# EBI-Metagenomics/deciphon-old

Measured on AMD Instinct MI355X. Metric: Gcell-updates/sec, higher is better.
Workload: dtype f32

## Files before the change

deciphon-old_amd/csrc/dcp_qlane.hip:

```cpp
#include "dcp_kernels.h"

#include <hip/hip_runtime.h>
#include <type_traits>

namespace
{
constexpr int NC = DCP_NCODES;

#ifndef DCP_QLANE_RECOMPUTE_B
#define DCP_QLANE_RECOMPUTE_B 1
#endif
constexpr bool kRecomputeB = DCP_QLANE_RECOMPUTE_B != 0;
#ifndef DCP_QLANE_WD
#define DCP_QLANE_WD 5
#endif
constexpr unsigned kWD = DCP_QLANE_WD;
constexpr unsigned kPlanes = kRecomputeB ? 3u : 4u;
#ifndef DCP_QLANE_DIAG
#define DCP_QLANE_DIAG 0
#endif

#ifndef DCP_QL_WPLANE
#define DCP_QL_WPLANE 1
#endif
#ifndef DCP_QL_IN16
#define DCP_QL_IN16 1
#endif
#ifndef DCP_QL_EM
#define DCP_QL_EM 1
#endif
constexpr bool kWPlane = DCP_QL_WPLANE != 0, kIn16 = DCP_QL_IN16 != 0, kEM = DCP_QL_EM != 0;

typedef float const __attribute__((address_space(4))) cfloat;
__device__ __forceinline__ cfloat *as_const(float const *p)
{
    return (cfloat *)(unsigned long long)p;
}

__device__ __forceinline__ float ninf() { return -__builtin_inff(); }
__device__ __forceinline__ float mx3(float a, float b, float c) { return fmaxf(fmaxf(a, b), c); }
__device__ __forceinline__ float mx5(float a, float b, float c, float d, float e)
{
    return mx3(mx3(a, b, c), d, e);
}

template <int G> struct QState
{
    float P[5][4 * G];
    float Q[5][4 * G];
    float PN[5], PR[5];
    float PJ[5], PC[5];
};

struct LaneXt
{
    float RR, SB, SN, NN, NB, ET, EC, CC, CT, EB, EJ, JJ, JB;
};

struct SweepOut
{
    float E, C, Rn;
};

template <int G> struct TileTrans
{
    float ent[4 * G], mi[4 * G], ii[4 * G];
    float mm[4 * G + 1], im[4 * G + 1], dm[4 * G + 1], md[4 * G + 1], dd[4 * G + 1];
};

template <int G> __device__ __forceinline__ void load_tile_trans(TileTrans<G> &t, cfloat *tt)
{
    constexpr int KT = 4 * G;
#pragma unroll
    for (int k = 0; k < KT; ++k)
    {
        t.ent[k] = tt[k * 8 + DCP_T_ENTRY];
        t.mi[k] = tt[k * 8 + DCP_T_MI];
        t.ii[k] = tt[k * 8 + DCP_T_II];
    }
#pragma unroll
    for (int k = 1; k <= KT; ++k)
    {
        t.mm[k] = tt[k * 8 + DCP_T_MM];
        t.im[k] = tt[k * 8 + DCP_T_IM];
        t.dm[k] = tt[k * 8 + DCP_T_DM];
        t.md[k] = tt[k * 8 + DCP_T_MD];
        t.dd[k] = tt[k * 8 + DCP_T_DD];
    }
    t.mm[0] = t.im[0] = t.dm[0] = t.md[0] = t.dd[0] = 0.0f;
}

struct RowIn
{
    float4 e0[5];
    float eI[5], eN[5];
};

template <int G, bool ROWS>
__device__ __forceinline__ void stage_tile_image(float *tabM, dcp_qlane_args const &a, dcp_ql_prof const &pm, unsigned t,
                                                 unsigned first, unsigned stride)
{
    constexpr unsigned N4 = (unsigned)(G * NC);
    float4 *dst = reinterpret_cast<float4 *>(tabM);
    if constexpr (!ROWS)
    {
        float4 const *__restrict__ src = reinterpret_cast<float4 const *>(a.emis_tiles + pm.tile_off + (size_t)t * (N4 * 4u));
        for (unsigned i = first; i < N4; i += stride)
            dst[i] = src[i];
    }
    else
    {
        float const *__restrict__ rows = a.emis_tiles + pm.tile_off + t * (4u * (unsigned)G);
        unsigned const ldk = pm.ldk, M = pm.core_size;
        for (unsigned i = first; i < N4; i += stride)
        {
            unsigned const grp = i / (unsigned)NC, code = i - grp * (unsigned)NC;
            float4 v = make_float4(ninf(), ninf(), ninf(), ninf());
            if (t * (4u * (unsigned)G) + grp * 4u < M)
                v = *reinterpret_cast<float4 const *>(rows + (size_t)code * ldk + grp * 4u);
            dst[i] = v;
        }
    }
}

__device__ __forceinline__ float ld_off(float const *base, unsigned boff)
{
    return *reinterpret_cast<float const *>(reinterpret_cast<char const *>(base) + boff);
}
typedef uint32_t const __attribute__((address_space(1))) *gu32_ptr;
typedef uint16_t const __attribute__((address_space(1))) *gu16_ptr;
typedef char const __attribute__((address_space(1))) *gchar_ptr;
__device__ __forceinline__ void st_off(float *base, unsigned boff, float v)
{
    *reinterpret_cast<float *>(reinterpret_cast<char *>(base) + boff) = v;
}

struct Ring
{
    float B[5], Xm[5], Xd[5], Em[5];
};

enum
{
    IO_HBM = 1,
    IO_LDS = 2
};
constexpr unsigned kRD = 16;
constexpr unsigned kRLanes = 256;
constexpr unsigned kRingPlaneBytes = kRD * kRLanes * 4u;
#ifndef DCP_Q2_SKEW
#define DCP_Q2_SKEW 4
#endif
#ifndef DCP_Q2_HYST
#define DCP_Q2_HYST 1
#endif
#ifndef DCP_Q2_SLEEP
#define DCP_Q2_SLEEP 2
#endif
#ifndef DCP_Q2_PRIO
#define DCP_Q2_PRIO 0
#endif
#ifndef DCP_Q2_STAGEMAP
#define DCP_Q2_STAGEMAP 1
#endif
constexpr unsigned kRingSkew = DCP_Q2_SKEW;
constexpr unsigned kRingHyst = DCP_Q2_HYST;
typedef float __attribute__((address_space(3))) lds_float;
typedef unsigned __attribute__((address_space(3))) lds_uint;

typedef char __attribute__((address_space(3))) lds_char;

struct LdsLink
{
    lds_char *base;
    unsigned my_flag;
    unsigned peer_flag;
    unsigned seen;
};
constexpr unsigned kL2TabIN = 43648u;
constexpr unsigned kL2FlagP = kL2TabIN + 2u * 1364u * 4u;
constexpr unsigned kL2FlagC = kL2FlagP + kRLanes * 4u;
constexpr unsigned kL2Null = kL2FlagC + kRLanes * 4u;
constexpr unsigned kL2Task = kL2Null + kRLanes * 4u;
constexpr unsigned kL2Abort = kL2Task + 4u;
constexpr unsigned kL2Err = kL2Task + 8u;
constexpr unsigned kL2Tab1 = 65536u;
constexpr unsigned kL2Ring = 7u * kRingPlaneBytes;
constexpr unsigned kL2Bytes = kL2Ring + 3u * kRingPlaneBytes;
static_assert(kL2Task + 16u <= kL2Tab1 && kL2Tab1 + kL2TabIN <= kL2Ring && kL2Bytes == 160u * 1024u, "LDS layout");
static_assert((kL2Ring & (kRingPlaneBytes - 1u)) == 0u, "ring slots are addressed by OR");
static_assert(kRD >= 12u, "a shorter ring can deadlock the two stages (five-row hand-shake groups)");

__device__ __forceinline__ void compiler_fence() { asm volatile("" ::: "memory"); }
#define DCP_ISA_MARK(name) asm volatile("; " name ::: "memory")
__device__ __forceinline__ unsigned flag_load(lds_uint *flag)
{
    return __hip_atomic_load(flag, __ATOMIC_RELAXED, __HIP_MEMORY_SCOPE_WORKGROUP);
}
__device__ __forceinline__ void flag_store(lds_uint *flag, unsigned v)
{
    __hip_atomic_store(flag, v, __ATOMIC_RELAXED, __HIP_MEMORY_SCOPE_WORKGROUP);
}
#ifndef DCP_Q2_BOUND
#define DCP_Q2_BOUND 1
#endif
constexpr unsigned kRingSpinBound = 1u << 23;
constexpr unsigned kRingPoison = 0x7fffff00u;
__device__ __forceinline__ unsigned ring_wait(LdsLink const &lk, unsigned need)
{
    lds_uint *flag = (lds_uint *)(lk.base + lk.peer_flag);
    unsigned v = __builtin_amdgcn_readfirstlane(flag_load(flag));
#if DCP_Q2_BOUND
    unsigned spins = 0;
#pragma nounroll
    while (v < need)
    {
        __builtin_amdgcn_s_sleep(DCP_Q2_SLEEP);
        v = __builtin_amdgcn_readfirstlane(flag_load(flag));
        if (__builtin_expect(++spins == kRingSpinBound, 0))
        {
            typedef unsigned __attribute__((address_space(1))) *gerr_ptr;
            gerr_ptr const err = *(gerr_ptr __attribute__((address_space(3))) *)(lk.base + kL2Err);
            __hip_atomic_store(err, 1u, __ATOMIC_RELAXED, __HIP_MEMORY_SCOPE_AGENT);
            flag_store((lds_uint *)(lk.base + kL2Abort), 1u);
            flag_store(flag, kRingPoison);
            v = kRingPoison;
            __builtin_amdgcn_s_waitcnt(0x0070);
        }
    }
#else
    while (v < need)
    {
        __builtin_amdgcn_s_sleep(DCP_Q2_SLEEP);
        v = __builtin_amdgcn_readfirstlane(flag_load(flag));
    }
#endif
    DCP_ISA_MARK("DCP_RING_ACQUIRED");
    return v;
}
__device__ __forceinline__ float ring_ld(LdsLink const &lk, unsigned rowoff, unsigned plane)
{
    return *(lds_float *)(lk.base + ((rowoff & (kRingPlaneBytes - 1u)) | kL2Ring) + plane * kRingPlaneBytes);
}
__device__ __forceinline__ void ring_st(LdsLink const &lk, unsigned rowoff, unsigned plane, float v)
{
    *(lds_float *)(lk.base + ((rowoff & (kRingPlaneBytes - 1u)) | kL2Ring) + plane * kRingPlaneBytes) = v;
}
__device__ __forceinline__ void ring_publish(LdsLink const &lk, unsigned rowoff, unsigned row)
{
    flag_store((lds_uint *)(lk.base + lk.my_flag + (rowoff & (kRLanes * 4u - 1u))), row);
}

template <bool FIRST>
__device__ __forceinline__ void ring_fetch_x(Ring &r, int slot, float const *pXm, float const *pXd,
                                             float const *pEm, unsigned off)
{
    if constexpr (!FIRST)
    {
        r.Xm[slot] = ld_off(pXm, off);
        r.Xd[slot] = ld_off(pXd, off);
        r.Em[slot] = ld_off(pEm, off);
    }
}
template <bool FIRST>
__device__ __forceinline__ void ring_fetch_b(Ring &r, int slot, float const *pB, unsigned off)
{
    if constexpr (!kRecomputeB && !FIRST) r.B[slot] = ld_off(pB, off);
}
template <bool FIRST>
__device__ __forceinline__ void ring_fetch(Ring &r, int slot, float const *pB, float const *pXm,
                                           float const *pXd, float const *pEm, unsigned off)
{
    ring_fetch_x<FIRST>(r, slot, pXm, pXd, pEm, off);
    ring_fetch_b<FIRST>(r, slot, pB, off);
}

struct GatherOff
{
    unsigned a[5];
};
template <unsigned BASE> struct GatherMasks
{
    unsigned base, m[4];
    __device__ __forceinline__ GatherMasks()
    {
        static_assert((BASE & 0x3fffu) == 0u, "the base must not overlap the window's 14 bits");
        base = BASE;
        if constexpr (BASE != 0u) asm volatile("" : "+s"(base));
#pragma unroll
        for (int l = 0; l < 4; ++l)
            m[l] = (((1u << (2 * l + 2)) - 1u) << 4) | base;
    }
};
template <unsigned BASE> __device__ __forceinline__ GatherOff gather_off(unsigned w, GatherMasks<BASE> const &gm)
{
    unsigned const wp = (DCP_QLANE_DIAG & 1) ? 0u : w;
    unsigned const w16 = kWPlane ? (BASE != 0u ? (wp | gm.base) : wp) : ((w << 4) | gm.base);
    GatherOff g;
#pragma unroll
    for (int l = 0; l < 4; ++l)
        g.a[l] = w16 & gm.m[l];
    if constexpr (kWPlane && BASE == 0u && !(DCP_QLANE_DIAG & 1)) asm volatile("v_mov_b32 %0, %1" : "=v"(g.a[4]) : "v"(w16));
    else g.a[4] = w16;
    return g;
}
template <int GROUP> __device__ __forceinline__ float4 gather_match(float const *tabM, GatherOff const &g, int l)
{
    constexpr unsigned first[5] = {0u, 4u, 20u, 84u, 340u};
    return *reinterpret_cast<float4 const *>(reinterpret_cast<char const *>(tabM) +
                                             (g.a[l] + (first[l] + (unsigned)GROUP * NC) * 16u));
}

template <int G, bool FIRST, bool LAST, bool IN16>
__device__ __forceinline__ void ql_fetch(RowIn &in, float const *tabM, float2 const *tabIN, GatherOff const &g)
{
    constexpr unsigned first[5] = {0u, 4u, 20u, 84u, 340u};
#pragma unroll
    for (int l = 0; l < 5; ++l)
    {
        in.e0[l] = gather_match<0>(tabM, g, l);
        float2 const v = *reinterpret_cast<float2 const *>(
            reinterpret_cast<char const *>(tabIN) + (IN16 ? g.a[l] + first[l] * 16u : (g.a[l] >> 1) + first[l] * 8u));
        in.eI[l] = v.x;
        in.eN[l] = v.y;
    }
}

template <int R> __device__ __forceinline__ float comp(float4 const &v)
{
    return R == 0 ? v.x : R == 1 ? v.y : R == 2 ? v.z : v.w;
}

template <int G, bool FIRST, bool LAST, int PH, int NT, int D, int IN = IO_HBM, int OUT = IO_HBM, unsigned TBASE = 0u,
          bool IN16 = kIn16>
__device__ __forceinline__ void ql_row(QState<G> &s, TileTrans<G> const &tr, float const *tabM,
                                       float2 const *tabIN, GatherOff &go,
                                       unsigned wn, RowIn &in, Ring &ring, float *pB, float *pXm,
                                       float *pXd, float *pEm, unsigned &off, LaneXt const &xt,
                                       bool live, bool at_end, bool &dirty, SweepOut &o,
                                       LdsLink const &lk, unsigned jrow, GatherMasks<TBASE> const &gm
#if DCP_QLANE_DIAG & 4
                                       , unsigned &off2, unsigned din
#endif
                                       )
{
    constexpr int KT = 4 * G;
    constexpr int s1 = (PH + 4) % 5, s2 = (PH + 3) % 5, s3 = (PH + 2) % 5, s4 = (PH + 1) % 5, s5 = PH;
    float const ni = ninf();

    static_assert(G <= 2, "gather_match<GROUP> is instantiated for groups 0 and 1");
    float4 e[G > 1 ? G - 1 : 1][5];
    if constexpr (G > 1)
    {
#pragma unroll
        for (int l = 0; l < 5; ++l)
            e[0][l] = gather_match<1>(tabM, go, l);
    }

    {
        constexpr int per_row = ((FIRST || IN != IO_HBM) ? 0 : 3) + ((LAST || OUT != IO_HBM) ? 0 : 3) +
                                ((!kRecomputeB && !FIRST) ? 1 : 0) + ((!kRecomputeB && FIRST) ? 1 : 0) + 1;
        constexpr int vm = ((D < (int)kWD ? D : (int)kWD) - 1) * per_row;
        constexpr int lgkm = G > 1 ? 5 : 0;
        __builtin_amdgcn_s_waitcnt((vm & 15) | ((vm >> 4) << 14) | (7 << 4) | (lgkm << 8));
    }
    __builtin_amdgcn_sched_barrier(0);
    float Xm = ni, Xd = ni, E = ni, Bj = ring.B[PH];
    if constexpr (!FIRST)
    {
        Xm = ring.Xm[PH];
        Xd = ring.Xd[PH];
        E = ring.Em[PH];
    }
    float eI[5], eN[5];
#pragma unroll
    for (int l = 0; l < 5; ++l)
    {
        eI[l] = in.eI[l];
        eN[l] = in.eN[l];
    }

    if constexpr (FIRST || kRecomputeB)
    {
        float const N = mx5(s.PN[s1] + eN[0], s.PN[s2] + eN[1], s.PN[s3] + eN[2],
                            s.PN[s4] + eN[3], s.PN[s5] + eN[4]);
        s.PN[PH] = N + xt.NN;
        Bj = N + xt.NB;
        if constexpr (FIRST)
        {
            float const Rn = mx5(s.PR[s1] + eN[0], s.PR[s2] + eN[1], s.PR[s3] + eN[2],
                                 s.PR[s4] + eN[3], s.PR[s5] + eN[4]);
            s.PR[PH] = Rn + xt.RR;
            o.Rn = at_end ? Rn : o.Rn;
            if constexpr (!kRecomputeB) st_off(pB, off, Bj);
        }
    }

    float pm = ni, pi = ni, pd = ni;
    float m_even = ni;
    auto node = [&](int k, float e0, float e1, float e2, float e3, float e4) {
        float const m = mx5(s.P[s1][k] + e0, s.P[s2][k] + e1, s.P[s3][k] + e2, s.P[s4][k] + e3,
                            s.P[s5][k] + e4);
        float const iv = mx5(s.Q[s1][k] + eI[0], s.Q[s2][k] + eI[1], s.Q[s3][k] + eI[2],
                             s.Q[s4][k] + eI[3], s.Q[s5][k] + eI[4]);
        float d, pin;
        if (k == 0)
        {
            d = Xd;
            pin = Xm;
        }
        else
        {
            d = fmaxf(pm + tr.md[k], pd + tr.dd[k]);
            pin = mx3(pm + tr.mm[k], pi + tr.im[k], pd + tr.dm[k]);
        }
        if constexpr (kEM)
        {
            if (k & 1) E = mx3(E, m_even, m);
            else m_even = m;
        }
        else E = mx3(E, m, d);
        s.P[PH][k] = fmaxf(Bj + tr.ent[k], pin);
        s.Q[PH][k] = fmaxf(m + tr.mi[k], iv + tr.ii[k]);
        pm = m, pi = iv, pd = d;
    };

    node(0, in.e0[0].x, in.e0[1].x, in.e0[2].x, in.e0[3].x, in.e0[4].x);
    node(1, in.e0[0].y, in.e0[1].y, in.e0[2].y, in.e0[3].y, in.e0[4].y);
    node(2, in.e0[0].z, in.e0[1].z, in.e0[2].z, in.e0[3].z, in.e0[4].z);
    node(3, in.e0[0].w, in.e0[1].w, in.e0[2].w, in.e0[3].w, in.e0[4].w);

    if constexpr (!FIRST && IN == IO_HBM)
    {
        asm volatile("" : "+v"(off) : "v"(E));
#if DCP_QLANE_DIAG & 4
        ring_fetch_x<FIRST>(ring, (PH + D) % 5, pXm + din, pXd + din, pEm + din, off);
#else
        ring_fetch_x<FIRST>(ring, (PH + D) % 5, pXm + D * NT, pXd + D * NT, pEm + D * NT, off);
#endif
    }

    __builtin_amdgcn_s_waitcnt(0xC07F | (0 << 8));
    go = gather_off<TBASE>(wn, gm);
    ql_fetch<G, FIRST, LAST, IN16>(in, tabM, tabIN, go);
    if constexpr (!FIRST && IN == IO_LDS)
    {
        constexpr int sl = (PH + 1) % 5;
        DCP_ISA_MARK("DCP_RING_TAKE");
        unsigned const nxt = off + kRLanes * 4u;
        ring.Xm[sl] = ring_ld(lk, nxt, 0);
        ring.Xd[sl] = ring_ld(lk, nxt, 1);
        ring.Em[sl] = ring_ld(lk, nxt, 2);
        DCP_ISA_MARK("DCP_RING_TAKEN");
        ring_publish(lk, off, jrow + 1u);
        DCP_ISA_MARK("DCP_RING_TAKE_END");
    }

#pragma unroll
    for (int g = 1; g < G; ++g)
    {
        float4 const *eg = e[g - 1];
        node(4 * g + 0, eg[0].x, eg[1].x, eg[2].x, eg[3].x, eg[4].x);
        node(4 * g + 1, eg[0].y, eg[1].y, eg[2].y, eg[3].y, eg[4].y);
        node(4 * g + 2, eg[0].z, eg[1].z, eg[2].z, eg[3].z, eg[4].z);
        node(4 * g + 3, eg[0].w, eg[1].w, eg[2].w, eg[3].w, eg[4].w);
    }

    if constexpr (!kRecomputeB && !FIRST)
    {
        asm volatile("" : "+v"(off) : "v"(pm));
        ring_fetch_b<FIRST>(ring, (PH + D) % 5, pB + D * NT, off);
    }

    if constexpr (!LAST)
    {
        float const oXm = mx3(pm + tr.mm[KT], pi + tr.im[KT], pd + tr.dm[KT]);
        float const oXd = fmaxf(pm + tr.md[KT], pd + tr.dd[KT]);
        if constexpr (OUT == IO_LDS)
        {
            DCP_ISA_MARK("DCP_RING_DATA");
            ring_st(lk, off, 0, oXm);
            ring_st(lk, off, 1, oXd);
            ring_st(lk, off, 2, E);
            DCP_ISA_MARK("DCP_RING_FLAG");
            ring_publish(lk, off, jrow);
            DCP_ISA_MARK("DCP_RING_DATA_END");
        }
        else
        {
#if DCP_QLANE_DIAG & 4
            unsigned const offw = off2;
#else
            unsigned const offw = off;
#endif
            st_off(pXm, offw, oXm);
            st_off(pXd, offw, oXd);
            st_off(pEm, offw, E);
        }
    }
    else
    {
        float const J = mx5(s.PJ[s1] + eN[0], s.PJ[s2] + eN[1], s.PJ[s3] + eN[2], s.PJ[s4] + eN[3],
                            s.PJ[s5] + eN[4]);
        float const C = mx5(s.PC[s1] + eN[0], s.PC[s2] + eN[1], s.PC[s3] + eN[2], s.PC[s4] + eN[3],
                            s.PC[s5] + eN[4]);
        float const B1 = fmaxf(E + xt.EB, J + xt.JB);
        dirty = dirty || (live && B1 > Bj);
        s.PJ[PH] = fmaxf(E + xt.EJ, J + xt.JJ);
        s.PC[PH] = fmaxf(E + xt.EC, C + xt.CC);
        o.E = at_end ? E : o.E;
        o.C = at_end ? C : o.C;
    }
}

template <int G, bool FIRST, bool LAST, int NT, int D, int IN = IO_HBM, int OUT = IO_HBM, unsigned TBASE = 0u,
          bool IN16 = kIn16>
__device__ __forceinline__ void ql_sweep(cfloat *tt, float const *tabM, float2 const *tabIN,
                                         uint32_t const *__restrict__ wordsT, unsigned rowbase,
                                         unsigned L, unsigned Lwave, bool active, float *sc,
                                         size_t plane, unsigned tid, LaneXt const &xt, bool &dirty,
                                         SweepOut &o, LdsLink lk
#if DCP_QLANE_DIAG & 4
                                         , unsigned tile_odd
#endif
                                         )
{
    constexpr int KT = 4 * G;
#if DCP_QLANE_DIAG & 4
    unsigned const rowstep = tile_odd ? 0u : (unsigned)NT;
    unsigned const rowstep_out = tile_odd ? (unsigned)NT : 0u;
    unsigned const din = (unsigned)D * rowstep;
    unsigned off2 = tid * 4u;
#else
    constexpr unsigned rowstep = (DCP_QLANE_DIAG & 2) ? 0u : (unsigned)NT;
#endif
    float const ni = ninf();
    TileTrans<G> tr;
    load_tile_trans<G>(tr, tt);
    QState<G> s;
#pragma unroll
    for (int h = 0; h < 5; ++h)
    {
#pragma unroll
        for (int k = 0; k < KT; ++k)
            s.P[h][k] = ni, s.Q[h][k] = ni;
        s.PN[h] = ni, s.PR[h] = ni, s.PJ[h] = ni, s.PC[h] = ni;
    }
    {
        float const B0 = 0.0f + xt.SB;
#pragma unroll
        for (int k = 0; k < KT; ++k)
            s.P[0][k] = B0 + tr.ent[k];
        s.PN[0] = 0.0f + xt.SN;
        s.PR[0] = 0.0f;
    }
    float *pXm = sc, *pXd = sc + plane, *pEm = sc + 2 * plane, *pB = sc + (kRecomputeB ? 0 : 3) * plane;
    unsigned off = (rowbase * (unsigned)NT + tid) * 4u;

    unsigned j = 1;
    static_assert(kWPlane, "the packed-word sequence planes are gone (round 4): a slot's groups are addressed by plane row");
    typedef uint16_t wq_t;
    wq_t wq[5];
    unsigned w;
    unsigned lane2 = tid * 2u;
    gu16_ptr const wpl = (gu16_ptr)wordsT + (size_t)rowbase * (unsigned)NT;
    asm volatile("" : "+v"(lane2));
    {
        w = wpl[NT + tid];
#pragma unroll
        for (int r = 2; r < 7; ++r)
            wq[r % 5] = wpl[r * NT + tid];
        __builtin_amdgcn_sched_barrier(0);
        __builtin_amdgcn_s_waitcnt(0x0F70);
    }
    RowIn in;
    Ring ring;
#pragma unroll
    for (int l = 0; l < 5; ++l)
    {
        in.e0[l] = float4{ni, ni, ni, ni}, in.eI[l] = ni, in.eN[l] = ni;
        ring.B[l] = ring.Xm[l] = ring.Xd[l] = ring.Em[l] = ni;
    }
    GatherMasks<TBASE> const gm;
    GatherOff go = gather_off<TBASE>(w, gm);
    ql_fetch<G, FIRST, LAST, IN16>(in, tabM, tabIN, go);
    if constexpr (!FIRST && IN == IO_LDS)
    {
        static_assert(NT == (int)kRLanes, "the ring's row stride is the scratch planes' row stride");
        unsigned const need0 = rowbase + (Lwave < kRingSkew ? Lwave : kRingSkew);
        lk.seen = ring_wait(lk, need0);
        DCP_ISA_MARK("DCP_RING_TAKE");
        ring.Xm[1] = ring_ld(lk, off, 0);
        ring.Xd[1] = ring_ld(lk, off, 1);
        ring.Em[1] = ring_ld(lk, off, 2);
        DCP_ISA_MARK("DCP_RING_TAKEN");
        ring_publish(lk, off, rowbase + 1u);
        DCP_ISA_MARK("DCP_RING_TAKE_END");
    }
    else
    {
        lk.seen = 0u;
#pragma unroll
        for (int r = 0; r < D; ++r)
            ring_fetch<(FIRST || IN != IO_HBM)>(ring, (r + 1) % 5, pB, pXm, pXd, pEm, off + (unsigned)r * rowstep * 4u);
    }

#if DCP_QLANE_DIAG & 8
#ifndef DCP_QLANE_DIAG_ROWS
#define DCP_QLANE_DIAG_ROWS 256u
#endif
#define QL_DIAG8_WRAP off &= (DCP_QLANE_DIAG_ROWS * (unsigned)NT * 4u - 1u);
#else
#define QL_DIAG8_WRAP
#endif
#if DCP_QLANE_DIAG & 4
#define QL_DIAG4_ARGS , off2, din
#define QL_DIAG4_STEP off2 += rowstep_out * 4u;
#else
#define QL_DIAG4_ARGS
#define QL_DIAG4_STEP
#endif
#define QL_ROW(PH)                                                                         \
    {                                                                                      \
                                                 \
        unsigned const pos = j + 1u;                                                       \
        ql_row<G, FIRST, LAST, PH, NT, D, IN, OUT, TBASE, IN16>(s, tr, tabM, tabIN, go,              \
                                   (unsigned)wq[(PH + 1) % 5], in, ring, pB, pXm,                    \
                                   pXd, pEm, off, xt, active && j <= L, active && j == L,  \
                                   dirty, o, lk, rowbase + j, gm QL_DIAG4_ARGS);           \
        {    \
             \
             \
             \
             \
            gu16_ptr wrow = wpl + (pos + 5u) * (unsigned)NT;                                     \
            asm volatile("" : "+s"(wrow));                                                   \
            asm volatile("" : "+v"(lane2));  \
            wq[(PH + 1) % 5] = *(gu16_ptr)((gchar_ptr)wrow + lane2);                          \
        }                                                                                    \
        off += rowstep * 4u;                                                                     \
        QL_DIAG8_WRAP                                                                            \
        QL_DIAG4_STEP                                                                            \
        ++j;                                                                               \
             \
             \
             \
        __builtin_amdgcn_sched_barrier(6);                                                 \
    }
    auto ring_sync = [&](unsigned n) {
        if constexpr (!FIRST && IN == IO_LDS)
        {
            unsigned const need = rowbase + (j + n < Lwave ? j + n : Lwave);
            if (lk.seen < need) lk.seen = ring_wait(lk, need + kRingHyst < rowbase + Lwave ? need + kRingHyst : rowbase + Lwave);
        }
        if constexpr (!LAST && OUT == IO_LDS)
        {
            unsigned const last = rowbase + j + n - 1u;
            if (last > lk.seen + kRD) lk.seen = ring_wait(lk, last - kRD + kRingHyst);
        }
    };
    while (j + 4 <= Lwave)
    {
        ring_sync(5u);
        QL_ROW(1) QL_ROW(2) QL_ROW(3) QL_ROW(4) QL_ROW(0)
    }
    ring_sync(4u);
    if (j <= Lwave) QL_ROW(1)
    if (j <= Lwave) QL_ROW(2)
    if (j <= Lwave) QL_ROW(3)
    if (j <= Lwave) QL_ROW(4)
#undef QL_ROW
}

template <bool IN16>
__device__ __forceinline__ void fill_tab_in(float *tab, float const *__restrict__ gi, float const *__restrict__ gn, unsigned t,
                                            unsigned nthreads)
{
    for (unsigned i = t; i < (unsigned)NC; i += nthreads)
    {
        if constexpr (IN16) *reinterpret_cast<float4 *>(tab + 4u * i) = float4{gi[i], gn[i], 0.0f, 0.0f};
        else *reinterpret_cast<float2 *>(tab + 2u * i) = float2{gi[i], gn[i]};
    }
}

typedef dcp_ql_group const __attribute__((address_space(4))) cgroup;
typedef uint32_t const __attribute__((address_space(4))) cu32;

struct GroupLane
{
    unsigned q, L, Lwave, rowbase;
    bool has;
    LaneXt xt;
};
__device__ __forceinline__ void load_group(dcp_qlane_args const &a, unsigned gi, unsigned lane, GroupLane &g)
{
    cgroup *gd = (cgroup *)(unsigned long long)(a.groups + gi);
    unsigned const qfirst = gd->qfirst, nq = gd->nq;
    g.rowbase = gd->rowbase;
    g.has = lane < nq;
    g.q = g.has ? a.qorder[qfirst + lane] : 0u;
    g.L = g.has ? a.seq_len[g.q] : 0u;
    g.Lwave = gd->lmax;
    float const *__restrict__ x = a.xtrans + (size_t)g.q * DCP_XSTRIDE;
    g.xt.RR = x[DCP_X_RR], g.xt.SB = x[DCP_X_SB], g.xt.SN = x[DCP_X_SN], g.xt.NN = x[DCP_X_NN];
    g.xt.NB = x[DCP_X_NB], g.xt.ET = x[DCP_X_ET], g.xt.EC = x[DCP_X_EC], g.xt.CC = x[DCP_X_CC];
    g.xt.CT = x[DCP_X_CT], g.xt.EB = x[DCP_X_EB], g.xt.EJ = x[DCP_X_EJ], g.xt.JJ = x[DCP_X_JJ];
    g.xt.JB = x[DCP_X_JB];
    __builtin_amdgcn_s_waitcnt(0x0F70);
    __builtin_amdgcn_sched_barrier(0);
}
__device__ __forceinline__ unsigned park_off(GroupLane const &g, unsigned NT, unsigned col)
{
    return ((g.rowbase + g.Lwave + 8u) * NT + col) * 4u;
}

__device__ __forceinline__ void ql_publish(dcp_qlane_args const &a, dcp_ql_prof const &pm, unsigned q, float nul, float alt,
                                           bool redo)
{
    if (redo)
    {
        unsigned const cls = pm.cls;
        unsigned const i = atomicAdd(a.redo_n + cls, 1u);
        if (i < a.redo_cap[cls]) a.redo[a.redo_base[cls] + i] = dcp_pair{q, pm.rs_slot};
        else *a.redo_overflow = 1u;
        return;
    }
    size_t const oi = (size_t)q * a.nprof_total + pm.pidx;
    if (a.out_null) a.out_null[oi] = nul;
    if (a.out_alt) a.out_alt[oi] = alt;
    if (dcp_lrt_hit(nul, alt, a.lrt_threshold))
    {
        unsigned const h = atomicAdd(a.nhits, 1u);
        if (h < a.hit_cap) a.hits[h] = dcp_hit{a.q_base + q, pm.pidx, nul, alt};
    }
}

}

template <int G, int NT, int D, bool ROWS = false>
__global__ __launch_bounds__(NT, NT / 128) void viterbi_qlane_kernel(dcp_qlane_args a)
{
    constexpr int KT = 4 * G;
    constexpr int TAB_FLOATS = G * NC * 4;
    __shared__ __attribute__((aligned(16))) float lds[TAB_FLOATS + (kIn16 ? 4 : 2) * NC];
    __shared__ unsigned s_task;
    float *tabM = lds;
    float2 *tabIN = reinterpret_cast<float2 *>(lds + TAB_FLOATS);
    unsigned const tid = threadIdx.x;
    size_t const plane = (size_t)a.plane_rows * (unsigned)NT;
    float *const sc = a.scratch + (size_t)blockIdx.x * kPlanes * plane;
    constexpr unsigned SLOTS = (unsigned)NT / 64u;

    for (;;)
    {
        if (tid == 0) s_task = atomicAdd(a.task_counter, 1u);
        __syncthreads();
        unsigned const task = __builtin_amdgcn_readfirstlane(s_task);
        __syncthreads();
        if (task >= a.ntasks) break;
        unsigned const slot = a.nprof - 1u - task / a.nqblocks;
        unsigned const qb = task % a.nqblocks;
        dcp_ql_prof const pm = a.profs[slot];
        unsigned const T = pm.ntiles;
        unsigned const sidx = __builtin_amdgcn_readfirstlane(qb * SLOTS + (tid >> 6));
        cu32 *sf = (cu32 *)(unsigned long long)a.slot_first;
        unsigned const g0 = sf[sidx], g1 = sf[sidx + 1u];
        uint32_t const *__restrict__ wordsT = a.words_t + __builtin_amdgcn_readfirstlane(a.wt_off[qb]);

        {
            float const *__restrict__ gi = a.emis_insert + (size_t)pm.pidx * NC;
            float const *__restrict__ gn = a.emis_null + (size_t)pm.pidx * NC;
            fill_tab_in<kIn16>(lds + TAB_FLOATS, gi, gn, tid, (unsigned)NT);
        }

        GroupLane g;
        bool const single = g1 - g0 == 1u;
        bool t_loaded = false;
        for (unsigned t = 0; t < T; ++t)
        {
            __syncthreads();
            stage_tile_image<G, ROWS>(tabM, a, pm, t, tid, (unsigned)NT);
            __syncthreads();
            cfloat *tt = as_const(a.ttrans + pm.ttrans_off + (size_t)t * (KT + 1) * 8);
            bool const first = t == 0, last = t + 1 == T;
            for (unsigned gi = g0; gi < g1; ++gi)
            {
                if (!(single && t_loaded)) load_group(a, gi, tid & 63u, g);
                t_loaded = true;
                if (g.Lwave == 0u) continue;
                SweepOut o{ninf(), ninf(), ninf()};
                bool dirty = false;
#if DCP_QLANE_DIAG & 4
#define QL_DIAG4_TILE , (t & 1u)
#else
#define QL_DIAG4_TILE
#endif
#define QL_SWEEP(F, L_)                                                                          \
    ql_sweep<G, F, L_, NT, D>(tt, tabM, tabIN, wordsT, g.rowbase, g.L, g.Lwave, g.has, sc, plane, tid, g.xt, dirty, o, LdsLink{} QL_DIAG4_TILE)
                if (first && last) QL_SWEEP(true, true);
                else if (first) QL_SWEEP(true, false);
                else if (last) QL_SWEEP(false, true);
                else QL_SWEEP(false, false);
#undef QL_SWEEP
                unsigned const po = park_off(g, (unsigned)NT, tid);
                if (first && !last) st_off(sc, po, o.Rn);
                if (last && g.has)
                {
                    float const nul = first ? o.Rn : ld_off(sc, po);
                    ql_publish(a, pm, g.q, nul, fmaxf(o.E + g.xt.ET, o.C + g.xt.CT), dirty || (kEM && pm.needs_exact_e));
                }
            }
        }
    }
}

template <int G, int D, bool ROWS = false>
__global__ __launch_bounds__(512, 2) void viterbi_qlane2_kernel(dcp_qlane_args a)
{
    constexpr int NT = (int)kRLanes;
    constexpr int KT = 4 * G;
    __shared__ __attribute__((aligned(16))) float lds[kL2Bytes / 4u];
    unsigned const wv = threadIdx.x >> 6;
#if DCP_Q2_STAGEMAP == 0
    unsigned const stage = __builtin_amdgcn_readfirstlane(wv & 1u);
    unsigned const tid = ((wv >> 1) << 6) | (threadIdx.x & 63u);
#else
    unsigned const stage = __builtin_amdgcn_readfirstlane(wv >> 2);
    unsigned const tid = threadIdx.x & 255u;
#endif
    unsigned *const s_task_p = reinterpret_cast<unsigned *>(lds + kL2Task / 4u);
    float *const tabM = lds + (stage ? kL2Tab1 / 4u : 0u);
    size_t const plane = (size_t)a.plane_rows * (unsigned)NT;
    float *const sc = a.scratch + (size_t)blockIdx.x * kPlanes * plane;
    constexpr unsigned SLOTS = (unsigned)NT / 64u;

#if DCP_Q2_PRIO == 1
    if (stage == 1u) __builtin_amdgcn_s_setprio(1);
#elif DCP_Q2_PRIO == 2
    if (stage == 0u) __builtin_amdgcn_s_setprio(1);
#endif
    LdsLink lk;
    lk.base = (lds_char *)lds;
    lk.my_flag = stage == 0u ? kL2FlagP : kL2FlagC;
    lk.peer_flag = (stage == 0u ? kL2FlagC : kL2FlagP) + (tid & ~63u) * 4u;
    lk.seen = 0u;
    if (threadIdx.x == 0) *(unsigned **)(lds + kL2Err / 4u) = a.ring_error;
    unsigned *const s_abort_p = reinterpret_cast<unsigned *>(lds + kL2Abort / 4u);

    for (;;)
    {
        if (threadIdx.x == 0)
        {
            unsigned const failed = __hip_atomic_load(a.ring_error, __ATOMIC_RELAXED, __HIP_MEMORY_SCOPE_AGENT);
            unsigned const next = atomicAdd(a.task_counter, 1u);
            *s_task_p = failed ? 0xffffffffu : next;
            *s_abort_p = 0u;
        }
        __syncthreads();
        unsigned const task = __builtin_amdgcn_readfirstlane(*s_task_p);
        __syncthreads();
        if (task >= a.ntasks) break;
        unsigned const slot = a.nprof - 1u - task / a.nqblocks;
        unsigned const qb = task % a.nqblocks;
        dcp_ql_prof const pm = a.profs[slot];
        unsigned const T = pm.ntiles;
        unsigned const sidx = __builtin_amdgcn_readfirstlane(qb * SLOTS + (tid >> 6));
        cu32 *sf = (cu32 *)(unsigned long long)a.slot_first;
        unsigned const g0 = sf[sidx], g1 = sf[sidx + 1u];
        uint32_t const *__restrict__ wordsT = a.words_t + __builtin_amdgcn_readfirstlane(a.wt_off[qb]);
        {
            float const *__restrict__ gi = a.emis_insert + (size_t)pm.pidx * NC;
            float const *__restrict__ gn = a.emis_null + (size_t)pm.pidx * NC;
            fill_tab_in<false>(lds + kL2TabIN / 4u, gi, gn, threadIdx.x, 512u);
        }
        bool const stalled = a.ring_stall != 0u && task == 0u && stage == 0u;

        unsigned const nsteps = (T + 1u) / 2u;
        unsigned const final_stage = (T - 1u) & 1u;
        GroupLane g;
        bool const single = g1 - g0 == 1u;
        bool t_loaded = false;
        for (unsigned st = 0; st < nsteps; ++st)
        {
            unsigned const t = 2u * st + stage;
            bool const mine = t < T;
            __syncthreads();
            if (mine) stage_tile_image<G, ROWS>(tabM, a, pm, t, tid, (unsigned)NT);
            flag_store((lds_uint *)(lk.base + lk.my_flag + tid * 4u), 0u);
            __syncthreads();
            if (!mine || (stalled && st == 0u) || __builtin_amdgcn_readfirstlane(*s_abort_p) != 0u) continue;
            cfloat *tt = as_const(a.ttrans + pm.ttrans_off + (size_t)t * (KT + 1) * 8);
            bool const first = t == 0u, last = t + 1u == T;
#if DCP_QLANE_DIAG & 4
#error "the two-stage kernel has no DIAG=4 build"
#endif
            for (unsigned gi = g0; gi < g1; ++gi)
            {
                if (!(single && t_loaded)) load_group(a, gi, tid & 63u, g);
                t_loaded = true;
                if (g.Lwave == 0u) continue;
                SweepOut o{ninf(), ninf(), ninf()};
                bool dirty = false;
#define QL2_SWEEP(F, L_, IN_, OUT_, TB_)                                                                  \
    ql_sweep<G, F, L_, NT, D, IN_, OUT_, TB_, false>(tt, lds, reinterpret_cast<float2 const *>(lds + (kL2TabIN - TB_ / 2u) / 4u), \
                                              wordsT, g.rowbase, g.L, g.Lwave, g.has, sc, plane, tid, g.xt, dirty, o, lk)
                if (stage == 0u)
                {
                    if (first && last) QL2_SWEEP(true, true, IO_HBM, IO_HBM, 0u);
                    else if (first) QL2_SWEEP(true, false, IO_HBM, IO_LDS, 0u);
                    else if (last) QL2_SWEEP(false, true, IO_HBM, IO_HBM, 0u);
                    else QL2_SWEEP(false, false, IO_HBM, IO_LDS, 0u);
                }
                else
                {
                    if (last) QL2_SWEEP(false, true, IO_LDS, IO_HBM, kL2Tab1);
                    else QL2_SWEEP(false, false, IO_LDS, IO_HBM, kL2Tab1);
                }
#undef QL2_SWEEP
                unsigned const po = park_off(g, (unsigned)NT, tid);
                if (first) st_off(sc, po, o.Rn);
                if (last)
                {
                    st_off(sc + plane, po, fmaxf(o.E + g.xt.ET, o.C + g.xt.CT));
                    st_off(sc + 2 * plane, po, dirty ? 1.0f : 0.0f);
                }
            }
        }
        __syncthreads();

        if (stage != final_stage) continue;
        for (unsigned gi = g0; gi < g1; ++gi)
        {
            cgroup *gd = (cgroup *)(unsigned long long)(a.groups + gi);
            GroupLane ge;
            ge.rowbase = gd->rowbase, ge.Lwave = gd->lmax;
            if (ge.Lwave == 0u || (tid & 63u) >= gd->nq) continue;
            unsigned const q = a.qorder[gd->qfirst + (tid & 63u)];
            unsigned const po = park_off(ge, (unsigned)NT, tid);
            float const nul = ld_off(sc, po), alt = ld_off(sc + plane, po);
            bool const dirty = ld_off(sc + 2 * plane, po) != 0.0f;
            ql_publish(a, pm, q, nul, alt, dirty || (kEM && pm.needs_exact_e));
        }
    }
}

template <int G, int D, bool ROWS = false>
__global__ __launch_bounds__(192, 1) void viterbi_qlane_w3_kernel(dcp_qlane_args a)
{
    constexpr int NT = 64;
    constexpr int KT = 4 * G;
    constexpr int TAB_FLOATS = G * NC * 4;
    constexpr int SLICE = TAB_FLOATS + 2 * NC;
    __shared__ __attribute__((aligned(16))) float lds[3 * SLICE];
    unsigned const wv = __builtin_amdgcn_readfirstlane(threadIdx.x >> 6);
    unsigned const tid = threadIdx.x & 63u;
    float *const tabM = lds + wv * SLICE;
    float2 *const tabIN = reinterpret_cast<float2 *>(tabM + TAB_FLOATS);
    size_t const plane = (size_t)a.plane_rows * (unsigned)NT;
    float *const sc = a.scratch + ((size_t)blockIdx.x * 3u + wv) * kPlanes * plane;

    for (;;)
    {
        unsigned t0 = 0;
        if (tid == 0) t0 = atomicAdd(a.task_counter, 1u);
        unsigned const task = __builtin_amdgcn_readfirstlane(t0);
        if (task >= a.ntasks) break;
        unsigned const slot = a.nprof - 1u - task / a.nqblocks;
        unsigned const qb = task % a.nqblocks;
        dcp_ql_prof const pm = a.profs[slot];
        unsigned const T = pm.ntiles;
        cu32 *sf = (cu32 *)(unsigned long long)a.slot_first;
        unsigned const g0 = sf[qb], g1 = sf[qb + 1u];
        uint32_t const *__restrict__ wordsT = a.words_t + __builtin_amdgcn_readfirstlane(a.wt_off[qb]);
        {
            float const *__restrict__ gi = a.emis_insert + (size_t)pm.pidx * NC;
            float const *__restrict__ gn = a.emis_null + (size_t)pm.pidx * NC;
            for (unsigned i = tid; i < (unsigned)NC; i += (unsigned)NT)
                tabIN[i] = float2{gi[i], gn[i]};
        }
        GroupLane g;
        bool const single = g1 - g0 == 1u;
        bool t_loaded = false;
        for (unsigned t = 0; t < T; ++t)
        {
            stage_tile_image<G, ROWS>(tabM, a, pm, t, tid, (unsigned)NT);
            compiler_fence();
            cfloat *tt = as_const(a.ttrans + pm.ttrans_off + (size_t)t * (KT + 1) * 8);
            bool const first = t == 0, last = t + 1 == T;
            for (unsigned gi = g0; gi < g1; ++gi)
            {
                if (!(single && t_loaded)) load_group(a, gi, tid, g);
                t_loaded = true;
                if (g.Lwave == 0u) continue;
                SweepOut o{ninf(), ninf(), ninf()};
                bool dirty = false;
#define QLW_SWEEP(F, L_)                                                                                  \
    ql_sweep<G, F, L_, NT, D, IO_HBM, IO_HBM, 0u, false>(tt, tabM, tabIN, wordsT, g.rowbase, g.L, g.Lwave, g.has, sc, plane, tid, g.xt, dirty, o, LdsLink{})
                if (first && last) QLW_SWEEP(true, true);
                else if (first) QLW_SWEEP(true, false);
                else if (last) QLW_SWEEP(false, true);
                else QLW_SWEEP(false, false);
#undef QLW_SWEEP
                unsigned const po = park_off(g, (unsigned)NT, tid);
                if (first && !last) st_off(sc, po, o.Rn);
                if (last && g.has)
                {
                    float const nul = first ? o.Rn : ld_off(sc, po);
                    ql_publish(a, pm, g.q, nul, fmaxf(o.E + g.xt.ET, o.C + g.xt.CT), dirty || (kEM && pm.needs_exact_e));
                }
            }
            compiler_fence();
        }
    }
}

template <int NT>
__global__ __launch_bounds__(NT) void transpose_words_kernel(dcp_qlane_args a)
{
    unsigned const qb = blockIdx.x, tid = threadIdx.x;
    unsigned const rows = (a.wt_off[qb + 1] - a.wt_off[qb]) * 2u / (unsigned)NT;
    uint16_t *dst = reinterpret_cast<uint16_t *>(a.words_t + a.wt_off[qb]);
    unsigned const sidx = qb * ((unsigned)NT / 64u) + (tid >> 6);
    unsigned const g0 = a.slot_first[sidx], g1 = a.slot_first[sidx + 1u];
    unsigned r = 0;
    for (unsigned gi = g0; gi < g1; ++gi)
    {
        dcp_ql_group const g = a.groups[gi];
        bool const has = (tid & 63u) < g.nq;
        unsigned const q = has ? a.qorder[g.qfirst + (tid & 63u)] : 0u;
        uint32_t const *__restrict__ src = a.seq_words + a.seq_woff[q];
        unsigned const len = has ? a.seq_len[q] : 0u;
        for (; r < g.rowbase; ++r)
            dst[r * (unsigned)NT + tid] = 0;
        unsigned w = 0, word = 0;
        unsigned const gr = g.lmax + 10u;
        for (unsigned k = 0; k < gr && r < rows; ++k, ++r)
        {
            if (k >= 1u)
            {
                unsigned const pos = k - 1u;
                if ((pos & 15u) == 0u) word = pos < len ? src[pos >> 4] : 0u;
                w = ((w << 2) | ((pos < len ? word >> ((pos & 15u) * 2u) : 0u) & 3u)) & 1023u;
            }
            dst[r * (unsigned)NT + tid] = (uint16_t)(w << 4);
        }
    }
    for (; r < rows; ++r)
        dst[r * (unsigned)NT + tid] = 0;
}

template <int G, int NT, int D>
static void launch_ql(dcp_qlane_args const *a, unsigned nblocks, hipStream_t s)
{
    if (a->tiles_from_rows) hipLaunchKernelGGL((viterbi_qlane_kernel<G, NT, D, true>), dim3(nblocks), dim3(NT), 0, s, *a);
    else hipLaunchKernelGGL((viterbi_qlane_kernel<G, NT, D>), dim3(nblocks), dim3(NT), 0, s, *a);
}

#ifndef DCP_QLANE_NT
#define DCP_QLANE_NT 256
#endif
#ifndef DCP_QLANE_D
#define DCP_QLANE_D 3
#endif
extern "C" unsigned dcp_qlane_block_size(void) { return DCP_QLANE_NT; }
extern "C" unsigned dcp_qlane_tile_nodes(void) { return 8u; }
extern "C" unsigned dcp_qlane_scratch_planes(void) { return kPlanes; }
extern "C" unsigned dcp_qlane_diag_build(void) { return DCP_QLANE_DIAG; }
extern "C" unsigned dcp_qlane_group_rows(unsigned lmax) { return (lmax + 11u) & ~1u; }
extern "C" unsigned dcp_qlane_window_planes(void) { return kWPlane ? 1u : 0u; }
extern "C" unsigned dcp_qlane_exact_e_by_redo(void) { return kEM ? 1u : 0u; }

extern "C" int dcp_launch_qlane_transpose(dcp_qlane_args const *a, unsigned nt, void *stream)
{
    if (nt == 64) hipLaunchKernelGGL((transpose_words_kernel<64>), dim3(a->nqblocks), dim3(64), 0, (hipStream_t)stream, *a);
    else if (nt == DCP_QLANE_NT)
        hipLaunchKernelGGL((transpose_words_kernel<DCP_QLANE_NT>), dim3(a->nqblocks), dim3(DCP_QLANE_NT), 0, (hipStream_t)stream, *a);
    else return 1;
    return 0;
}

extern "C" unsigned dcp_qlane2_lds_bytes(void) { return kL2Bytes; }

extern "C" int dcp_launch_qlane_w3(dcp_qlane_args const *a, unsigned nblocks, void *stream)
{
    if (a->tiles_from_rows)
        hipLaunchKernelGGL((viterbi_qlane_w3_kernel<2, DCP_QLANE_D, true>), dim3(nblocks), dim3(192), 0, (hipStream_t)stream, *a);
    else hipLaunchKernelGGL((viterbi_qlane_w3_kernel<2, DCP_QLANE_D>), dim3(nblocks), dim3(192), 0, (hipStream_t)stream, *a);
    return 0;
}

extern "C" int dcp_launch_qlane2(dcp_qlane_args const *a, unsigned nblocks, void *stream)
{
    if (a->tiles_from_rows)
        hipLaunchKernelGGL((viterbi_qlane2_kernel<2, DCP_QLANE_D, true>), dim3(nblocks), dim3(512), 0, (hipStream_t)stream, *a);
    else hipLaunchKernelGGL((viterbi_qlane2_kernel<2, DCP_QLANE_D>), dim3(nblocks), dim3(512), 0, (hipStream_t)stream, *a);
    return 0;
}

extern "C" int dcp_launch_qlane(dcp_qlane_args const *a, unsigned nblocks, unsigned nt, void *stream)
{
    if (nt == DCP_QLANE_NT) launch_ql<2, DCP_QLANE_NT, DCP_QLANE_D>(a, nblocks, (hipStream_t)stream);
    else return 1;
    return 0;
}
```

Measured before the change: 1421.

## Prefetch next tile's emission image into registers during the current sweep

Replaces the synchronous stage_tile_image load into LDS with a register-staged prefetch. The image for tile t+2 is issued into per-lane float4 registers after the current tile's sweep and written to LDS at the next step. The goal is to hide global-load latency behind the sweep and the barrier. The cost is more VGPRs, which can lower occupancy or cause spills. Separately, peer_flag is made wave-uniform with readfirstlane so it can live in a scalar register.

```diff
diff --git a/deciphon-old_amd/csrc/dcp_qlane.hip b/deciphon-old_amd/csrc/dcp_qlane.hip
--- a/deciphon-old_amd/csrc/dcp_qlane.hip
+++ b/deciphon-old_amd/csrc/dcp_qlane.hip
@@ -249,6 +249,91 @@
 __device__ __forceinline__ void ring_publish(LdsLink const &lk, unsigned rowoff, unsigned row)
 {
     flag_store((lds_uint *)(lk.base + lk.my_flag + (rowoff & (kRLanes * 4u - 1u))), row);
+}
+
+template <int G> struct TileRegs
+{
+    static constexpr unsigned N4 = (unsigned)(G * NC), PER_LANE = (N4 + kRLanes - 1u) / kRLanes;
+    float4 v[PER_LANE];
+};
+struct ImgSrc
+{
+    float const *tables;
+    dcp_ql_prof const __attribute__((address_space(4))) *prof;
+    unsigned wave64;
+    __device__ __forceinline__ float const *base() const { return tables + prof->tile_off; }
+    __device__ __forceinline__ unsigned ldk() const { return prof->ldk; }
+    __device__ __forceinline__ unsigned M() const { return prof->core_size; }
+};
+__device__ __forceinline__ ImgSrc img_src(dcp_qlane_args const &a, unsigned slot, unsigned tid)
+{
+    ImgSrc r;
+    r.tables = a.emis_tiles;
+    r.prof = (dcp_ql_prof const __attribute__((address_space(4))) *)(unsigned long long)(a.profs + slot);
+    r.wave64 = __builtin_amdgcn_readfirstlane(tid & ~63u);
+    return r;
+}
+__device__ __forceinline__ unsigned img_lane(ImgSrc const &src)
+{
+    unsigned lane;
+    asm volatile("v_mbcnt_lo_u32_b32 %0, -1, 0\n\tv_mbcnt_hi_u32_b32 %0, -1, %0" : "=&v"(lane));
+    return lane + src.wave64;
+}
+template <int G, bool ROWS>
+__device__ __forceinline__ void issue_tile_image(TileRegs<G> &r, ImgSrc const &is, unsigned t)
+{
+    constexpr unsigned N4 = TileRegs<G>::N4, PER = TileRegs<G>::PER_LANE;
+    unsigned const tid = img_lane(is);
+    DCP_ISA_MARK("DCP_IMG_LOADS");
+    if constexpr (!ROWS)
+    {
+        char const *src = reinterpret_cast<char const *>(is.base() + (size_t)t * (N4 * 4u));
+#pragma unroll
+        for (unsigned k = 0; k < PER; ++k)
+        {
+            unsigned const i = tid + k * kRLanes;
+            r.v[k] = *reinterpret_cast<float4 const *>(src + ((k + 1u) * kRLanes <= N4 || i < N4 ? i : tid) * 16u);
+        }
+    }
+    else
+    {
+        char const *rows = reinterpret_cast<char const *>(is.base() + t * (4u * (unsigned)G));
+        unsigned const ldk = is.ldk(), M = is.M();
+#pragma unroll
+        for (unsigned k = 0; k < PER; ++k)
+        {
+            unsigned const i = tid + k * kRLanes;
+            unsigned const grp = i / (unsigned)NC, code = i - grp * (unsigned)NC;
+            bool const there = i < N4 && t * (4u * (unsigned)G) + grp * 4u < M;
+            r.v[k] = *reinterpret_cast<float4 const *>(rows + (there ? (code * ldk + grp * 4u) * 4u : 0u));
+        }
+    }
+    __builtin_amdgcn_sched_barrier(0);
+    DCP_ISA_MARK("DCP_IMG_LOADS_END");
+}
+template <int G> __device__ __forceinline__ void drop_tile_image(TileRegs<G> &r)
+{
+#pragma unroll
+    for (unsigned k = 0; k < TileRegs<G>::PER_LANE; ++k)
+        asm volatile("" : "=v"(r.v[k].x), "=v"(r.v[k].y), "=v"(r.v[k].z), "=v"(r.v[k].w));
+}
+template <int G, bool ROWS>
+__device__ __forceinline__ void store_tile_image(float *tabM, TileRegs<G> const &r, ImgSrc const &is, unsigned t)
+{
+    constexpr unsigned N4 = TileRegs<G>::N4, PER = TileRegs<G>::PER_LANE;
+    float4 *dst = reinterpret_cast<float4 *>(tabM);
+    unsigned const tid = img_lane(is);
+#pragma unroll
+    for (unsigned k = 0; k < PER; ++k)
+    {
+        unsigned const i = tid + k * kRLanes;
+        float4 v = r.v[k];
+        if constexpr (ROWS)
+        {
+            if (!(t * (4u * (unsigned)G) + (i / (unsigned)NC) * 4u < is.M())) v = make_float4(ninf(), ninf(), ninf(), ninf());
+        }
+        if ((k + 1u) * kRLanes <= N4 || i < N4) dst[i] = v;
+    }
 }
 
 template <bool FIRST>
@@ -842,7 +927,7 @@
     LdsLink lk;
     lk.base = (lds_char *)lds;
     lk.my_flag = stage == 0u ? kL2FlagP : kL2FlagC;
-    lk.peer_flag = (stage == 0u ? kL2FlagC : kL2FlagP) + (tid & ~63u) * 4u;
+    lk.peer_flag = __builtin_amdgcn_readfirstlane((stage == 0u ? kL2FlagC : kL2FlagP) + (tid & ~63u) * 4u);
     lk.seen = 0u;
     if (threadIdx.x == 0) *(unsigned **)(lds + kL2Err / 4u) = a.ring_error;
     unsigned *const s_abort_p = reinterpret_cast<unsigned *>(lds + kL2Abort / 4u);
@@ -880,15 +965,25 @@
         GroupLane g;
         bool const single = g1 - g0 == 1u;
         bool t_loaded = false;
+        TileRegs<G> img;
+        ImgSrc const isrc = img_src(a, slot, tid);
+        if (stage < T) issue_tile_image<G, ROWS>(img, isrc, stage);
+        else drop_tile_image<G>(img);
         for (unsigned st = 0; st < nsteps; ++st)
         {
             unsigned const t = 2u * st + stage;
             bool const mine = t < T;
             __syncthreads();
-            if (mine) stage_tile_image<G, ROWS>(tabM, a, pm, t, tid, (unsigned)NT);
+            if (mine && (!(DCP_QLANE_DIAG & 16) || st == 0u)) store_tile_image<G, ROWS>(tabM, img, isrc, t);
             flag_store((lds_uint *)(lk.base + lk.my_flag + tid * 4u), 0u);
             __syncthreads();
-            if (!mine || (stalled && st == 0u) || __builtin_amdgcn_readfirstlane(*s_abort_p) != 0u) continue;
+            bool const more = !(DCP_QLANE_DIAG & 16) && t + 2u < T;
+            if (!mine || (stalled && st == 0u) || __builtin_amdgcn_readfirstlane(*s_abort_p) != 0u)
+            {
+                if (more) issue_tile_image<G, ROWS>(img, isrc, t + 2u);
+                else drop_tile_image<G>(img);
+                continue;
+            }
             cfloat *tt = as_const(a.ttrans + pm.ttrans_off + (size_t)t * (KT + 1) * 8);
             bool const first = t == 0u, last = t + 1u == T;
 #if DCP_QLANE_DIAG & 4
@@ -925,6 +1020,8 @@
                     st_off(sc + 2 * plane, po, dirty ? 1.0f : 0.0f);
                 }
             }
+            if (more) issue_tile_image<G, ROWS>(img, isrc, t + 2u);
+            else drop_tile_image<G>(img);
         }
         __syncthreads();
 
```

Result: no change. 1423 (median of 2 runs) (+0.1%).
